# SewoongLab/PLeaS-Merging

Measured on AMD Instinct MI355X. Metric: wall-clock (s): ResNet-101 pair, 100-batch act-match + 400-step PLeaS, 1/8 GPU, lower is better.
Workload: dtype f32

## Files before the change

include/pleas_hip.h:

```cpp
#ifndef PLEAS_HIP_H
#define PLEAS_HIP_H

#include <stddef.h>
#include <stdint.h>

#ifdef __cplusplus
extern "C" {
#endif

#define PLEAS_OK 0
#define PLEAS_EINVAL (-22)
#define PLEAS_ENOMEM (-12)
#define PLEAS_EHIP (-5)

const char* pleas_version(void);
const char* pleas_last_error(void);

#define PLEAS_EPI_INNER 0
#define PLEAS_EPI_NEG_CDIST 1
size_t pleas_gram_ws_bytes(int B, int C, int64_t HW);
int pleas_gram_accum(const float* x, const float* y, int B, int C, int64_t HW, int epilogue, int accumulate,
                     float* acc, void* ws, size_t ws_bytes, void* stream);

typedef struct pleas_gram_node {
// ... 6 lines not shown
    int derived;
    int source;
    const float* scale_x;
    const float* shift_x;
    const float* scale_y;
    const float* shift_y;
} pleas_gram_node;
size_t pleas_gram_batch_ws_bytes(const pleas_gram_node* nodes, int n_nodes, const int* group_C, int n_groups);
int pleas_gram_batch(const pleas_gram_node* nodes, int n_nodes, float* const* group_acc, const int* group_C,
                     int n_groups, int epilogue, int accumulate, void* ws, size_t ws_bytes, int ws_fresh, void* stream);

#define PLEAS_LSAP_MAX_N 4096
int pleas_lsap_batched(const float* const* cost, const int* n, int nprob, int maximize, int64_t* const* col_ind,
                       void* stream);
int pleas_lsap_host(const void* cost, int is_double, int n, int maximize, int64_t* col_ind);

size_t pleas_bottleneck_ws_bytes(const int* n, int nprob);
int pleas_bottleneck_batched(const float* const* cost, const int* n, int nprob, int maximize, int64_t* const* col_ind,
                             float* t_out, void* ws, size_t ws_bytes, void* stream);
int pleas_bottleneck_host(const void* cost, int is_double, int n, int maximize, int64_t* col_ind, double* t_out);

int pleas_merge_blocks(const float* w1, const float* w2, float* out, int64_t outer, int rows_out, int cols_out,
                       int64_t inner, int rows_src, int cols_src, const int32_t* row1, const int32_t* row2,
                       const int32_t* col1, const int32_t* col2, int n_merged_rows, void* stream);

typedef struct pleas_merge_item {
    const float* w1;
    const float* w2;
    float* out;
    const int32_t* row1;
    const int32_t* row2;
    int64_t outer, inner;
    int rows_out, rows_src, n_merged;
    int sub_stride, sub_h, sub_w;
} pleas_merge_item;
size_t pleas_merge_batch_ws_bytes(const pleas_merge_item* items, int n_items);
int pleas_merge_batch(const pleas_merge_item* items, int n_items, void* ws, size_t ws_bytes, int ws_fresh, void* stream);

int pleas_bn_act(const float* x, const float* scale, const float* shift, const float* res, float* y, int64_t n,
                 int channels, int64_t inner, int relu, void* stream);
int pleas_bn_act_tracked(const float* x, const float* scale, const float* shift, const float* res, float* y_bn,
                         float* y_sum, float* y, int64_t n, int channels, int64_t inner, int relu, void* stream);

int pleas_bn_act_tracked_batches(const float* x, const float* scale, const float* shift, const float* res, float* y_bn,
                                 float* y_sum, float* y, int64_t n_per_batch, int batches, int channels, int64_t inner,
                                 int relu, void* stream);

int pleas_bn_act_maxpool(const float* x, const float* scale, const float* shift, float* y, int64_t n, int channels, int H,
                         int W, int KH, int KW, int stride, int pad, int relu, void* stream);

size_t pleas_bn_train_ws_bytes(int64_t n, int channels);
int pleas_bn_train_fold(const float* x, int64_t n, int channels, int64_t inner, const float* gamma, const float* beta,
                        double eps, double momentum, float* running_mean, float* running_var,
                        int64_t* num_batches_tracked, float* scale, float* shift, void* ws, size_t ws_bytes,
                        void* stream);
int pleas_bn_train_fold_batches(const float* x, int64_t n, int batches, int channels, int64_t inner, const float* gamma,
                                const float* beta, double eps, double momentum, float* running_mean, float* running_var,
                                int64_t* num_batches_tracked, float* scale, float* shift, void* ws, size_t ws_bytes,
                                void* stream);

int pleas_masked_adam(float* p, const float* g, const float* mask, float* m, float* v, int64_t n, float lr,
                      float b1, float b2, float eps, int step, void* stream);

size_t pleas_sqerr_ws_bytes(int64_t n);
int pleas_sqerr(const float* a, const float* b, int64_t n, float scale, int accumulate, float* out, float dscale,
                float* diff, void* ws, size_t ws_bytes, void* stream);

int pleas_channel_sum(const float* x, int N, int C, int64_t HW, float* out, void* stream);

typedef struct pleas_fwd_layer {
    const float* ip;
    const float* w;
    const float* bias;
    const float* o1;
    const float* o2;
    const int32_t* row1;
    const int32_t* row2;
    float* resid;
    int N, Cout, Cin, Hin, Win, KH, KW, stride, pad, Csrc, n_merged;
    float dscale, loss_scale;
    int flags;
} pleas_fwd_layer;
#define PLEAS_FWD_KPOS_MAJOR 1
size_t pleas_fwd_batch_ws_bytes(const pleas_fwd_layer* layers, int n_layers);
int pleas_fwd_plan_lanes(double* form_ms, int* form_lane, int* form_items);
int pleas_fwd_plan_units(const pleas_fwd_layer* layers, int n_layers, const double* form_ms, int* units, int max_units);
int pleas_fwd_batch(const pleas_fwd_layer* layers, int n_layers, float* loss, void* ws, size_t ws_bytes, int ws_fresh,
                    void* stream);
int pleas_conv2d_fwd(const float* x, const float* w, const float* bias, float* y, int N, int Cin, int Hin, int Win, int Cout,
                     int KH, int KW, int stride, int pad, int flags, void* stream);
int pleas_conv2d_bn_act_fwd(const float* x, const float* w, const float* bias, float* y, const float* scale,
                            const float* shift, const float* res, float* z, int relu, int N, int Cin, int Hin, int Win,
                            int Cout, int KH, int KW, int stride, int pad, int flags, void* stream);
typedef struct pleas_wgrad_layer {
    const float* resid;
    const float* ip;
    float* grad;
    int N, Cout, Cin, Hin, Win, KH, KW, stride, pad;
    int flags;
} pleas_wgrad_layer;
#define PLEAS_WGRAD_ACCUMULATE 1
#define PLEAS_WGRAD_KPOS_MAJOR 2
int pleas_target_residual(const float* out, const float* o1, const float* o2, const int32_t* row1, const int32_t* row2,
                          int n_merged, int N, int C, int Csrc, int64_t HW, float dscale, float* resid, float* partials,
                          int* n_partials, void* stream);
int pleas_target_residual_max_partials(void);
int pleas_loss_final(const float* partials, const int* n_partials, const float* scale, int stride, int n_layers,
                     float* loss, void* stream);
size_t pleas_wgrad_batch_ws_bytes(const pleas_wgrad_layer* layers, int n_layers);
int pleas_wgrad_batch(const pleas_wgrad_layer* layers, int n_layers, void* ws, size_t ws_bytes, int ws_fresh,
                      void* stream);
int pleas_wgrad_plan_info(const pleas_wgrad_layer* layers, int n_layers, int* info);

int pleas_allreduce_sum(float* buf, int64_t n, void* comm, void* stream);

typedef struct pleas_neq_layer {
    const float* ip;
    float* A;
    int N, Cin, Hin, Win, KH, KW, stride, pad;
} pleas_neq_layer;
size_t pleas_normal_eq_ws_bytes(const pleas_neq_layer* layers, int n_layers);
int pleas_normal_eq_accum(const pleas_neq_layer* layers, int n_layers, void* ws, size_t ws_bytes, int ws_fresh,
                          void* stream);
int pleas_normal_eq_finalize(const pleas_neq_layer* layers, int n_layers, void* stream);
int pleas_normal_eq_plan_info(const pleas_neq_layer* layers, int n_layers, double* info);

int pleas_cholesky_solve_batched(float* const* A, float* const* Bt, const int* K, const int* N, int nprob, float lambda,
                                 int* info, void* stream);

void pleas_prof_enable(int on);
void pleas_prof_select(unsigned kernel_mask);
void pleas_prof_reset(void);
int pleas_prof_collect(int kernel, int64_t* launches, double* total_ms, double* flops, double* bytes);

void pleas_gram_tune(int target_blocks, int min_chunks_per_split);
void pleas_gram_batch_tune(int item_chunks, int xcd_order);
#define PLEAS_ARITH_FP32 0
#define PLEAS_ARITH_SPLIT_BF16 1
void pleas_arith(int mode);
int pleas_arith_get(void);
void pleas_gram_split_bf16(int on);
void pleas_wgrad_tune(int item_chunks);

#ifdef __cplusplus
}
#endif
#endif
```

pleas_merging_amd/csrc/conv_fwd.hip:

```cpp
#include <algorithm>
#include <mutex>
#include <vector>

#include "common.hpp"
#include "fwd_schedule.hpp"

namespace pleas {

typedef float f32x4 __attribute__((ext_vector_type(4)));
typedef float f32x16 __attribute__((ext_vector_type(16)));

constexpr int fBK = 32;
constexpr int fLdsA = 36;
constexpr int fLdsB = 36;
constexpr int fTN = 128;
constexpr int fThreads = 256;

struct FwdLayerDev {
    const float* ip;
    const float* w;
    const float* bias;
    const float* o1;
    const float* o2;
    const int32_t* row1;
// ... 692 lines not shown
        store_a((c + 1) & 1, ra_next);
        if (newb) {
            if constexpr (NBUF == 2) {
                bsel ^= 1;
                store_b(bsel, rb_next);
            } else {
                __syncthreads();
                store_b(0, rb0);
            }
        }
        __syncthreads();
        r1 = r2;
        cb1 = cb2;
    };
    int r = 0;
    int c = 0;
    for (; c + 2 < nchunks; c += 2) {
        const int ra_ = r1;
        step(c, r, ra1, ra0, rb1, rb0);
        const int rb_ = r1;
        step(c + 1, ra_, ra0, ra1, rb0, rb1);
        r = rb_;
    }
    if (c + 1 < nchunks) {
        const int ra_ = r1;
        step(c, r, ra1, ra0, rb1, rb0);
        r = ra_;
    }
    fwd_load_maps<TM, PLAIN>(L, i0, m1, m2, bias_v);
    compute((nchunks - 1) & 1, bsel, r);
    __syncthreads();
    fwd_epilogue<TM, PLAIN>(L, it, acc, m1, m2, bias_v, smem, partials);
}

struct FwdForm {
    bool flat;
    int tm;
    int sub;
    bool split;
    int occupancy[2];
    double weight;
};
constexpr int fForms = 10;
constexpr FwdForm kFwdForms[fForms] = {
    {false, 128, 4, false, {2, 2}, 2.5}, {false, 64, 4, false, {2, 2}, 2.5},
    {false, 128, 1, false, {2, 2}, 2.5}, {false, 64, 1, false, {2, 2}, 2.5},
    {true, 128, 0, true, {2, 2}, 1.0},   {true, 128, 1, false, {2, 2}, 2.0}, {true, 128, 2, true, {2, 2}, 1.0},
    {true, 64, 0, true, {2, 3}, 1.0},    {true, 64, 1, false, {2, 2}, 2.0},  {true, 64, 2, true, {2, 3}, 1.0},
};
constexpr int fwd_form_of(int variant) {
    if (variant & 8) return ((variant & 1) ? 7 : 4) + ((variant >> 4) & 3);
    return variant & 3;
}
constexpr bool fwd_forms_match_variants() {
    for (int f = 0; f < fForms; ++f) {
        const FwdForm& F = kFwdForms[f];
        const int variant = (F.tm == 64 ? 1 : 0) | (F.flat ? 8 | (F.sub << 4) : (F.sub == 1 ? 2 : 0));
        if (fwd_form_of(variant) != f || (F.split && !(F.flat && F.sub != 1))) return false;
    }
    return true;
}
static_assert(fwd_forms_match_variants(), "kFwdForms is indexed by the form id");
template <int FORM, int SPLIT = 0>
__global__ __launch_bounds__(fThreads, kFwdForms[FORM].occupancy[SPLIT]) void fwd_batch_kernel(const FwdLayerDev* __restrict__ layers,
                                                             const FwdItemDev* __restrict__ items,
                                                             float* __restrict__ partials) {
    extern __shared__ __attribute__((aligned(16))) float smem[];
    const FwdItemDev it = items[blockIdx.x];
    if (it.layer < 0) return;
    const FwdLayerDev L = layers[it.layer];
    constexpr FwdForm F = kFwdForms[FORM];
    if constexpr (F.flat) fwd_flat_tile<F.tm, F.sub, SPLIT>(L, it, smem, partials);
    else fwd_tile<F.tm, F.sub>(L, it, smem, partials);
}
template <int FORM, int SPLIT = 0, int BN = 0>
__global__ __launch_bounds__(fThreads, kFwdForms[FORM].occupancy[SPLIT]) void conv2d_fwd_kernel(const FwdLayerDev L, const int tms) {
    extern __shared__ __attribute__((aligned(16))) float smem[];
    const FwdItemDev it{0, (int)(blockIdx.x % (unsigned)tms), (int)(blockIdx.x / (unsigned)tms), 0};
    constexpr FwdForm F = kFwdForms[FORM];
    constexpr int PLAIN = 1 + BN;
    if constexpr (F.flat) fwd_flat_tile<F.tm, F.sub, SPLIT, PLAIN>(L, it, smem, nullptr);
    else fwd_tile<F.tm, F.sub, PLAIN>(L, it, smem, nullptr);
}
struct FwdFormKernels {
    void (*batch[2])(const FwdLayerDev*, const FwdItemDev*, float*);
    void (*conv2d[2][2])(const FwdLayerDev, const int);
};
template <int FORM>
static constexpr FwdFormKernels fwd_form_kernels() {
    constexpr int S = kFwdForms[FORM].split ? 1 : 0;
    return {{fwd_batch_kernel<FORM, 0>, fwd_batch_kernel<FORM, S>},
            {{conv2d_fwd_kernel<FORM, 0, 0>, conv2d_fwd_kernel<FORM, S, 0>}, {conv2d_fwd_kernel<FORM, 0, 1>, conv2d_fwd_kernel<FORM, S, 1>}}};
}
static const FwdFormKernels kFwdKernels[fForms] = {fwd_form_kernels<0>(), fwd_form_kernels<1>(), fwd_form_kernels<2>(), fwd_form_kernels<3>(),
                                                   fwd_form_kernels<4>(), fwd_form_kernels<5>(), fwd_form_kernels<6>(), fwd_form_kernels<7>(),
                                                   fwd_form_kernels<8>(), fwd_form_kernels<9>()};
constexpr int fLanes = 3;
static SideStreams<fLanes> g_fwd_side;

struct FwdLossDev {
    int begin, count;
    float scale;
    int pad;
};
__global__ __launch_bounds__(64) void fwd_loss_kernel(const float* __restrict__ partials, const FwdLossDev* __restrict__ ld,
                                                      float* __restrict__ loss) {
    const FwdLossDev d = ld[blockIdx.x];
    double s = 0.0;
    for (int i = threadIdx.x; i < d.count; i += 64) s += (double)partials[d.begin + i];
#pragma unroll
    for (int off = 32; off >= 1; off >>= 1) s += __shfl_xor(s, off);
    if (threadIdx.x == 0) loss[blockIdx.x] = (float)(s * (double)d.scale);
}

constexpr int fPtrBatch = 56;
struct FwdPtrBatch {
    int base, count;
    const float* ip[fPtrBatch];
    const float* w[fPtrBatch];
    const float* bias[fPtrBatch];
    const float* o1[fPtrBatch];
    const float* o2[fPtrBatch];
    const int32_t* row1[fPtrBatch];
    const int32_t* row2[fPtrBatch];
    float* resid[fPtrBatch];
};
__global__ void fwd_set_ptrs_kernel(FwdLayerDev* __restrict__ layers, const FwdPtrBatch b) {
    const int t = blockIdx.x * blockDim.x + threadIdx.x;
    if (t < b.count) {
        FwdLayerDev& L = layers[b.base + t];
        L.ip = b.ip[t];
        L.w = b.w[t];
        L.bias = b.bias[t];
        L.o1 = b.o1[t];
        L.o2 = b.o2[t];
        L.row1 = b.row1[t];
        L.row2 = b.row2[t];
        L.resid = b.resid[t];
    }
}

struct FwdPlan {
    std::vector<int64_t> key;
    std::vector<FwdLayerDev> layers;
    std::vector<FwdItemDev> items;
    std::vector<FwdLossDev> loss;
    size_t off_layers = 0, off_items = 0, off_loss = 0, off_parts = 0, total = 0;
    int form_begin[fForms] = {0}, form_count[fForms] = {0};
    size_t form_lds[fForms] = {0};
    std::vector<float> item_work;
    std::vector<FwdUnit> units;
    double flops = 0, bytes = 0;
    int n_parts = 0;
    bool uploaded = false;
    bool split = false;
    int launches = 0, calib = 0;
    hipEvent_t t0[kFwdMaxUnits], t1[kFwdMaxUnits];
    int timed = 0;
    bool timing_events() {
        if (timed == 0) {
            timed = 1;
            for (int u = 0; u < kFwdMaxUnits && timed == 1; ++u)
                if (hipEventCreate(&t0[u]) != hipSuccess || hipEventCreate(&t1[u]) != hipSuccess) timed = -1;
        }
        return timed == 1;
    }
// ... 83 lines not shown
        P.form_lds[form] = std::max(P.form_lds[form], lds_bytes);
        P.flops += 2.0 * l.Cout * (double)Kd * (double)Ptot;
        P.bytes += ((double)l.Cin * l.N * l.Hin * l.Win + 3.0 * l.Cout * (double)Ptot) * sizeof(float);
    }
    for (int f = 0; f < fForms; ++f) {
        P.form_begin[f] = (int)P.items.size();
        std::vector<FwdItemDev> part = xcd_order_items(work[f], FwdItemDev{-1, 0, 0, 0}, false);
        P.items.insert(P.items.end(), part.begin(), part.end());
        P.form_count[f] = (int)part.size();
    }
    P.item_work.assign(P.items.size(), 0.f);
    for (size_t k = 0; k < P.items.size(); ++k)
        if (P.items[k].layer >= 0) {
            const FwdLayerDev& d = P.layers[P.items[k].layer];
            P.item_work[k] = (float)(ceil_div(d.Kd, fBK) * kFwdForms[fwd_form_of(d.variant)].tm);
        }
    P.units.clear();
    for (int f = 0; f < fForms; ++f)
        if (P.form_count[f] > 0)
            P.units.push_back(FwdUnit{f, P.form_begin[f], P.form_count[f], 0, form_work[f] * kFwdForms[f].weight});
    fwd_deal_lanes(P.units, fLanes + 1);
    P.launches = P.calib = 0;
    P.n_parts = parts;
    size_t off = 0;
    P.off_layers = off;
    off = align256(off + P.layers.size() * sizeof(FwdLayerDev));
    P.off_items = off;
    off = align256(off + P.items.size() * sizeof(FwdItemDev));
    P.off_loss = off;
    off = align256(off + P.loss.size() * sizeof(FwdLossDev));
    P.off_parts = off;
    P.total = off + (size_t)parts * sizeof(float);
    P.uploaded = false;
    return PLEAS_OK;
}

}

using namespace pleas;

extern "C" int pleas_fwd_plan_lanes(double* form_ms, int* form_lane, int* form_items) {
    if (!form_ms || !form_lane || !form_items) return bad_arg("fwd_plan_lanes: null pointer");
    std::lock_guard<std::mutex> lk(g_fplan_mu);
    if (!g_fplans.last) return bad_arg("fwd_plan_lanes: no grouped forward has run yet");
    const FwdPlan& P = *g_fplans.last;
    for (int f = 0; f < fForms; ++f) {
        form_ms[f] = 0;
        form_lane[f] = 0;
        form_items[f] = P.form_count[f];
    }
    for (const auto& u : P.units) {
        form_ms[u.form] += u.ms;
        form_lane[u.form] = form_lane[u.form] * 10 + u.lane + 1;
    }
    return P.calib;
}

extern "C" int pleas_fwd_plan_units(const pleas_fwd_layer* layers, int n_layers, const double* form_ms, int* units, int max_units) {
    if (!layers || n_layers <= 0 || !units || max_units <= 0) return bad_arg("fwd_plan_units: empty layer list / null output");
    FwdPlan tmp;
    const int rc = build_fwd_plan(tmp, layers, n_layers);
    if (rc != PLEAS_OK) return rc;
    if (form_ms) {
        for (auto& u : tmp.units) u.ms = form_ms[u.form];
        (void)fwd_schedule_measured(tmp.units, tmp.form_items(), fLanes + 1, kFwdMaxUnits);
    }
    const int n = (int)std::min<size_t>(tmp.units.size(), (size_t)max_units);
    for (int i = 0; i < n; ++i) {
        units[4 * i + 0] = tmp.units[i].form;
        units[4 * i + 1] = tmp.units[i].begin;
        units[4 * i + 2] = tmp.units[i].count;
        units[4 * i + 3] = tmp.units[i].lane;
    }
    return (int)tmp.units.size();
}

extern "C" size_t pleas_fwd_batch_ws_bytes(const pleas_fwd_layer* layers, int n_layers) {
    if (!layers || n_layers <= 0) return 0;
    FwdPlan tmp;
    if (build_fwd_plan(tmp, layers, n_layers) != PLEAS_OK) return 0;
    return tmp.total;
}

static int conv2d_launch(const float* x, const float* w, const float* bias, float* y, const float* scale, const float* shift,
                         const float* res, float* z, int relu, int N, int Cin, int Hin, int Win, int Cout, int KH, int KW,
                         int stride, int pad, int flags, void* stream_) {
    if (!x || !w || !y) return bad_arg("conv2d_fwd: null pointer");
    if (((uintptr_t)w & 15) != 0 || ((uintptr_t)x & 15) != 0) return bad_arg("conv2d_fwd: x and w must be 16-byte aligned");
    const bool bn = scale != nullptr;
    if (bn && (!shift || !z)) return bad_arg("conv2d_bn_act_fwd: scale needs shift and z");
    if (bn && ((((uintptr_t)y | (uintptr_t)z | (uintptr_t)res) & 15) != 0))
        return bad_arg("conv2d_bn_act_fwd: y, z and res must be 16-byte aligned");
    pleas_fwd_layer l{};
    l.ip = x; l.w = w; l.bias = bias; l.resid = y;
    l.N = N; l.Cout = Cout; l.Cin = Cin; l.Hin = Hin; l.Win = Win; l.KH = KH; l.KW = KW; l.stride = stride; l.pad = pad;
    l.Csrc = 1; l.n_merged = 0; l.dscale = 1.f; l.loss_scale = 0.f; l.flags = flags;
    FwdLayerDev d{};
    size_t lds = 0;
    int TM = 128;
    if (const int rc = fwd_describe(l, d, lds, TM); rc != PLEAS_OK) return rc;
    d.ip = x; d.w = w; d.bias = bias; d.o1 = x; d.o2 = x; d.row1 = nullptr; d.row2 = nullptr; d.resid = y;
    d.part_base = 0;
    d.bn_scale = scale; d.bn_shift = shift; d.bn_res = res; d.bn_z = z; d.bn_relu = relu ? 1 : 0;
    const int tms = (int)ceil_div(Cout, TM), tps = (int)ceil_div((int64_t)d.Ptot, fTN);
    const dim3 grid((unsigned)((int64_t)tms * tps));
    hipStream_t st = (hipStream_t)stream_;
    const double out_floats = (double)Cout * d.Ptot;
    ProfScope prof(kProfConv2d, 2.0 * Cout * (double)d.Kd * (double)d.Ptot,
                   ((double)Cin * N * Hin * Win + out_floats * (bn ? (res ? 3.0 : 2.0) : 1.0)) * sizeof(float), st);
    hipLaunchKernelGGL(kFwdKernels[fwd_form_of(d.variant)].conv2d[bn ? 1 : 0][arith_mode() == 1 ? 1 : 0], grid, dim3(fThreads), lds, st, d, tms);
    PLEAS_LAUNCH_CHECK("conv2d_fwd_kernel");
    return PLEAS_OK;
}

extern "C" int pleas_conv2d_fwd(const float* x, const float* w, const float* bias, float* y, int N, int Cin, int Hin, int Win,
                                int Cout, int KH, int KW, int stride, int pad, int flags, void* stream_) {
    return conv2d_launch(x, w, bias, y, nullptr, nullptr, nullptr, nullptr, 0, N, Cin, Hin, Win, Cout, KH, KW, stride, pad, flags,
                         stream_);
}

extern "C" int pleas_conv2d_bn_act_fwd(const float* x, const float* w, const float* bias, float* y, const float* scale,
                                       const float* shift, const float* res, float* z, int relu, int N, int Cin, int Hin,
                                       int Win, int Cout, int KH, int KW, int stride, int pad, int flags, void* stream_) {
    if (!scale || !shift || !z) return bad_arg("conv2d_bn_act_fwd: null pointer");
    return conv2d_launch(x, w, bias, y, scale, shift, res, z, relu, N, Cin, Hin, Win, Cout, KH, KW, stride, pad, flags, stream_);
}

static void fwd_adopt_measurements(FwdPlan& P) {
    if (P.calib != 1) return;
    const int active = (int)P.units.size();
    bool ready = true;
    for (int u = 0; ready && u < active; ++u) ready = hipEventQuery(P.t1[u]) == hipSuccess;
    if (ready) {
        for (int u = 0; u < active; ++u) {
            float ms = 0.f;
            P.units[u].ms = hipEventElapsedTime(&ms, P.t0[u], P.t1[u]) == hipSuccess ? ms : 0.0;
        }
        P.calib = 2;
        if (fwd_schedule_measured(P.units, P.form_items(), fLanes + 1, kFwdMaxUnits))
            g_fcalib.publish(P.key, P.units);
    }
    (void)hipGetLastError();
}

static int fwd_launch_units(FwdPlan& P, const FwdLayerDev* dl, const FwdItemDev* items, float* parts, hipStream_t stream) {
    ProfScope prof(kProfConvFwd, P.flops, P.bytes, stream);
    SideStreams<fLanes>::Set& side = g_fwd_side.current();
    const int active = (int)P.units.size();
    const bool fork = active > 1 && side.ok;
    const bool measure = fork && P.calib == 0 && P.launches == kFwdCalibAt && active <= kFwdMaxUnits && P.timing_events();
    if (fork) PLEAS_HIP_CHECK(hipEventRecord(side.forked, stream));
    bool lane_used[fLanes + 1] = {false};
    for (int o = 0; o < active; ++o) {
        const FwdUnit& un = P.units[o];
        const int lane = fork ? un.lane : 0;
        hipStream_t st = lane == 0 ? stream : side.streams[lane - 1];
        if (lane > 0 && !lane_used[lane]) PLEAS_HIP_CHECK(hipStreamWaitEvent(st, side.forked, 0));
        lane_used[lane] = true;
        if (measure) PLEAS_HIP_CHECK(hipEventRecord(P.t0[o], st));
        hipLaunchKernelGGL(kFwdKernels[un.form].batch[P.split ? 1 : 0], dim3((unsigned)un.count), dim3(fThreads), P.form_lds[un.form], st,
                           dl, items + un.begin, parts);
        if (measure) PLEAS_HIP_CHECK(hipEventRecord(P.t1[o], st));
    }
    if (measure) P.calib = 1;
    for (int lane = 1; lane <= fLanes; ++lane)
        if (lane_used[lane]) {
            PLEAS_HIP_CHECK(hipEventRecord(side.joined[lane - 1], side.streams[lane - 1]));
            PLEAS_HIP_CHECK(hipStreamWaitEvent(stream, side.joined[lane - 1], 0));
        }
    return PLEAS_OK;
}

extern "C" int pleas_fwd_batch(const pleas_fwd_layer* layers, int n_layers, float* loss, void* ws, size_t ws_bytes,
                               int ws_fresh, void* stream_) {
    if (!layers || n_layers <= 0 || !loss) return bad_arg("conv_fwd: empty layer list");
    for (int i = 0; i < n_layers; ++i) {
        const pleas_fwd_layer& l = layers[i];
        if (!l.ip || !l.w || !l.o1 || !l.o2 || !l.row1 || !l.row2 || !l.resid) return bad_arg("conv_fwd: null pointer");
        if (((uintptr_t)l.w & 15) != 0) return bad_arg("conv_fwd: weights must be 16-byte aligned");
        if (((uintptr_t)l.ip & 15) != 0) return bad_arg("conv_fwd: the merged input must be 16-byte aligned");
    }
    hipStream_t stream = (hipStream_t)stream_;
    std::lock_guard<std::mutex> lk(g_fplan_mu);
    std::vector<int64_t> key;
    key.push_back(n_layers * 2 + arith_mode());
    key.push_back((int64_t)(uintptr_t)ws);
    for (int i = 0; i < n_layers; ++i) {
        const pleas_fwd_layer& l = layers[i];
        for (int v : {l.N, l.Cout, l.Cin, l.Hin, l.Win, l.KH, l.KW, l.stride, l.pad, l.Csrc, l.n_merged, l.flags})
            key.push_back(v);
        int32_t bits[2];
        std::memcpy(&bits[0], &l.dscale, 4);
// ... 45 lines not shown
```

pleas_merging_amd/hip_ops.py:

```python
from __future__ import annotations

import ctypes
import math
import threading
from typing import List, Optional, Sequence, Tuple

import numpy as np
import torch

from . import _lib
from ._lib import EPI_INNER, EPI_NEG_CDIST, PleasHipError, check


class _Pinned(threading.local):

    depth = 0
    handle = 0


_PINNED = _Pinned()


def _stream() -> int:
    if _PINNED.depth > 0:
# ... 581 lines not shown
    rc = _lib.lib().pleas_loss_final(partials.data_ptr(), n_partials.data_ptr(), scale.data_ptr(), stride, L,
                                     loss.data_ptr(), _stream())
    check(rc, "pleas_loss_final")


class MergeBatch(_GroupedLaunch):

    STRUCT, WS_BYTES, LAUNCH = _lib.MergeItem, "pleas_merge_batch_ws_bytes", "pleas_merge_batch"

    def add(self, w1: torch.Tensor, w2: torch.Tensor, row_axis: int, row1: torch.Tensor, row2: torch.Tensor,
            n_merged_rows: int, out: Optional[torch.Tensor] = None, subsample: int = 1) -> torch.Tensor:
        if w1.shape != w2.shape or not w1.is_cuda or w1.dtype != torch.float32 or w2.dtype != torch.float32:
            raise PleasHipError("MergeBatch.add: fp32 CUDA sources of equal shape expected")
        w1, w2 = w1.contiguous(), w2.contiguous()
        shape = list(w1.shape)
        row_axis = row_axis % w1.dim()
        rows_out = int(row1.numel())
        want = shape[:row_axis] + [rows_out] + shape[row_axis + 1:]
        sub = (0, 0, 0)
        if subsample > 1:
            if w1.dim() != 4 or row_axis != 1:
                raise PleasHipError("MergeBatch.add: subsample needs [N, C, H, W] sources merged along axis 1")
            sub = (int(subsample), shape[2], shape[3])
            want = want[:2] + [-(-shape[2] // subsample), -(-shape[3] // subsample)]
        if out is None:
            out = torch.empty(want, dtype=torch.float32, device=w1.device)
        elif list(out.shape) != want or out.dtype != torch.float32 or not out.is_contiguous() or out.device != w1.device:
            raise PleasHipError("MergeBatch.add: out must be a contiguous fp32 tensor of shape %s" % (want,))
        self._queue((w1, w2, out, row1, row2), (math.prod(shape[:row_axis]), math.prod(want[row_axis + 1:]), rows_out,
                                                shape[row_axis], int(n_merged_rows)) + sub)
        return out

    def _fill(self, a, tensors, geo) -> None:
        a.w1, a.w2, a.out, a.row1, a.row2 = (t.data_ptr() for t in tensors)
        a.outer, a.inner, a.rows_out, a.rows_src, a.n_merged, a.sub_stride, a.sub_h, a.sub_w = geo


def fwd_plan_lanes() -> dict:
    ms, lane, items = (ctypes.c_double * 10)(), (ctypes.c_int * 10)(), (ctypes.c_int * 10)()
    state = _lib.lib().pleas_fwd_plan_lanes(ms, lane, items)
    return {"state": state, "forms": {f: {"ms": round(ms[f], 4), "lane": lane[f], "items": items[f]} for f in range(10) if items[f]}}


class FwdBatch(_GroupedLaunch):

    STRUCT, WS_BYTES, LAUNCH = _lib.FwdLayer, "pleas_fwd_batch_ws_bytes", "pleas_fwd_batch"
    KPOS_MAJOR = 1

    def add(self, ip, w, bias, o1, o2, row1, row2, n_merged: int, resid, dscale: float, loss_scale: float,
            kernel=(1, 1), stride: int = 1, pad: int = 0, flags: int = 0) -> None:
        for t in (ip, w, o1, o2, resid):
            if not t.is_contiguous():
                raise PleasHipError("FwdBatch.add: contiguous tensors expected")
        N, Cin = ip.shape[0], ip.shape[1]
        Hin, Win = (ip.shape[2], ip.shape[3]) if ip.dim() == 4 else (1, 1)
        self._queue((ip, w, bias, o1, o2, row1, row2, resid),
                    (N, w.shape[0], Cin, Hin, Win, kernel[0], kernel[1], stride, pad, o1.shape[1], int(n_merged),
                     float(dscale), float(loss_scale), int(flags)))

    def _fill(self, a, tensors, geo) -> None:
        a.ip, a.w, a.bias, a.o1, a.o2, a.row1, a.row2, a.resid = (t.data_ptr() if t is not None else None for t in tensors)
        (a.N, a.Cout, a.Cin, a.Hin, a.Win, a.KH, a.KW, a.stride, a.pad, a.Csrc, a.n_merged, a.dscale, a.loss_scale,
         a.flags) = geo

    def _launch_args(self, loss: torch.Tensor) -> tuple:
        if loss.numel() != len(self._arr) or not loss.is_contiguous():
            raise PleasHipError("FwdBatch: loss must hold one float per layer")
        return (loss.data_ptr(),)

    def flush(self, loss: torch.Tensor) -> None:
        self._flush(loss)


def _conv_geometry(name: str, x: torch.Tensor, w: torch.Tensor, stride: int, pad: int, kpos_major: bool):
    if x.dim() != 4 or w.dim() != 4 or not x.is_contiguous() or not w.is_contiguous():
        raise PleasHipError("%s: contiguous 4-D tensors expected" % name)
    N, Cin, H, W = x.shape
    KH, KW = (w.shape[1], w.shape[2]) if kpos_major else (w.shape[2], w.shape[3])
    if (w.shape[3] if kpos_major else w.shape[1]) != Cin:
        raise PleasHipError("%s: %d input channels vs a weight of %s" % (name, Cin, tuple(w.shape)))
    return N, Cin, H, W, w.shape[0], KH, KW, (H + 2 * pad - KH) // stride + 1, (W + 2 * pad - KW) // stride + 1


def conv2d(x: torch.Tensor, w: torch.Tensor, bias: Optional[torch.Tensor], stride: int, pad: int, kpos_major: bool = False,
           out: Optional[torch.Tensor] = None) -> torch.Tensor:
    _need_gpu(x, w)
    N, Cin, H, W, Cout, KH, KW, Ho, Wo = _conv_geometry("conv2d", x, w, stride, pad, kpos_major)
    if out is None:
        out = torch.empty((N, Cout, Ho, Wo), dtype=torch.float32, device=x.device)
    check(_lib.lib().pleas_conv2d_fwd(x.data_ptr(), w.data_ptr(), bias.data_ptr() if bias is not None else None, out.data_ptr(),
                                      N, Cin, H, W, Cout, KH, KW, stride, pad, FwdBatch.KPOS_MAJOR if kpos_major else 0,
                                      _stream()), "pleas_conv2d_fwd")
    return out


def conv2d_bn_act(x: torch.Tensor, w: torch.Tensor, bias: Optional[torch.Tensor], stride: int, pad: int, kpos_major: bool,
                  scale: torch.Tensor, shift: torch.Tensor, res: Optional[torch.Tensor], relu: bool):
    _need_gpu(x, w, scale, shift)
    N, Cin, H, W, Cout, KH, KW, Ho, Wo = _conv_geometry("conv2d_bn_act", x, w, stride, pad, kpos_major)
    if scale.numel() != Cout or shift.numel() != Cout or scale.dtype != torch.float32 or shift.dtype != torch.float32:
        raise PleasHipError("conv2d_bn_act: scale / shift must be fp32 vectors of %d channels" % Cout)
    if res is not None and (tuple(res.shape) != (N, Cout, Ho, Wo) or res.dtype != torch.float32 or not res.is_contiguous()
                            or res.device != x.device):
        raise PleasHipError("conv2d_bn_act: the identity must be a contiguous fp32 tensor shaped like the output")
    y = torch.empty((N, Cout, Ho, Wo), dtype=torch.float32, device=x.device)
    z = torch.empty_like(y)
    check(_lib.lib().pleas_conv2d_bn_act_fwd(x.data_ptr(), w.data_ptr(), bias.data_ptr() if bias is not None else None,
                                             y.data_ptr(), scale.data_ptr(), shift.data_ptr(),
                                             res.data_ptr() if res is not None else None, z.data_ptr(), 1 if relu else 0,
                                             N, Cin, H, W, Cout, KH, KW, stride, pad,
                                             FwdBatch.KPOS_MAJOR if kpos_major else 0, _stream()), "pleas_conv2d_bn_act_fwd")
    return y, z


class WgradBatch(_GroupedLaunch):

    STRUCT, WS_BYTES, LAUNCH = _lib.WgradLayer, "pleas_wgrad_batch_ws_bytes", "pleas_wgrad_batch"
    ACCUMULATE, KPOS_MAJOR = 1, 2

    def add(self, resid: torch.Tensor, ip: torch.Tensor, grad: torch.Tensor, kernel=(1, 1), stride: int = 1,
            pad: int = 0, flags: int = 0) -> None:
        if not (resid.is_contiguous() and ip.is_contiguous() and grad.is_contiguous()):
            raise PleasHipError("WgradBatch.add: contiguous tensors expected")
        N, Cout, Cin = resid.shape[0], resid.shape[1], ip.shape[1]
        Hin, Win = (ip.shape[2], ip.shape[3]) if ip.dim() == 4 else (1, 1)
        self._queue((resid, ip, grad), (N, Cout, Cin, Hin, Win, kernel[0], kernel[1], stride, pad, flags))

    def _fill(self, a, tensors, geo) -> None:
        a.resid, a.ip, a.grad = (t.data_ptr() for t in tensors)
        a.N, a.Cout, a.Cin, a.Hin, a.Win, a.KH, a.KW, a.stride, a.pad, a.flags = geo

    @staticmethod
    def plan_info(geometries) -> List[dict]:
        geometries = list(geometries)
        n = len(geometries)
        if n == 0:
            return []
        arr = (_lib.WgradLayer * n)()
        for a, geo in zip(arr, geometries):
            a.N, a.Cout, a.Cin, a.Hin, a.Win, a.KH, a.KW, a.stride, a.pad, a.flags = (int(v) for v in geo)
        info = (ctypes.c_int * (6 * n))()
        check(_lib.lib().pleas_wgrad_plan_info(arr, n, info), "pleas_wgrad_plan_info")
        return [{"variant": info[6 * i], "S": info[6 * i + 1], "tiles_cout": info[6 * i + 2], "tiles_cin": info[6 * i + 3],
                 "items": info[6 * i + 4], "rows": bool(info[6 * i + 5])} for i in range(n)]

class NormalEqBatch(_GroupedLaunch):

    STRUCT, WS_BYTES, LAUNCH = _lib.NeqLayer, "pleas_normal_eq_ws_bytes", "pleas_normal_eq_accum"

    def __init__(self, device: torch.device):
        super().__init__(device)
        self._seen: dict = {}

    def add(self, ip: torch.Tensor, A: torch.Tensor, kernel=(1, 1), stride: int = 1, pad: int = 0) -> None:
        if not (ip.is_contiguous() and A.is_contiguous()):
            raise PleasHipError("NormalEqBatch.add: contiguous tensors expected")
        N, Cin = ip.shape[0], ip.shape[1]
        Hin, Win = (ip.shape[2], ip.shape[3]) if ip.dim() == 4 else (1, 1)
        K = kernel[0] * kernel[1] * Cin
        if tuple(A.shape) != (K, K):
            raise PleasHipError("NormalEqBatch.add: A must be (%d, %d)" % (K, K))
        geo = (N, Cin, Hin, Win, kernel[0], kernel[1], stride, pad)
        self._queue((ip, A), geo)
        self._seen[A.data_ptr()] = (A, geo)

    def _fill(self, a, tensors, geo) -> None:
        ip, A = tensors
        a.ip, a.A = (ip.data_ptr() if ip is not None else 0), A.data_ptr()
        a.N, a.Cin, a.Hin, a.Win, a.KH, a.KW, a.stride, a.pad = geo

    def _layer_array(self, pairs):
        arr = (_lib.NeqLayer * len(pairs))()
        for a, (A, geo) in zip(arr, pairs):
            self._fill(a, (None, A), geo)
        return arr

    def seen(self) -> dict:
        return dict(self._seen)

    def finalize(self, pairs=None) -> None:
        pairs = list(self._seen.values()) if pairs is None else list(pairs)
        if pairs:
            check(_lib.lib().pleas_normal_eq_finalize(self._layer_array(pairs), len(pairs), _stream()),
                  "pleas_normal_eq_finalize")

    def plan_info(self) -> dict:
        pairs = list(self._seen.values())
        info = (ctypes.c_double * 4)()
        if pairs:
            check(_lib.lib().pleas_normal_eq_plan_info(self._layer_array(pairs), len(pairs), info), "pleas_normal_eq_plan_info")
        return {"flops": info[0], "flops_executed": info[1], "items": int(info[2]), "blocks_to_finalize": int(info[3])}


def cholesky_solve_batched(As: Sequence[torch.Tensor], Bts: Sequence[torch.Tensor], ridge: float = 0.0) -> torch.Tensor:
# ... 39 lines not shown
```

Before: 5.857.

## Add persistent weight-resident streaming kernel for 1x1 conv forward

Adds a persistent conv2d forward kernel for 1x1 flat convolutions with Cin up to 256. It keeps a whole Cout tile of weights in LDS and streams pixel tiles through a double-buffered register and LDS pipeline, with the bias/BN/residual/ReLU epilogue fused in. The grid is sized to the number of resident workgroups from an occupancy query, so weights are loaded once per workgroup rather than once per tile. The aim is to cut repeated weight traffic and launch tail effects. The cost is heavy LDS use, lower occupancy, and a path that is on by default for matching shapes.

```diff
diff --git a/include/pleas_hip.h b/include/pleas_hip.h
--- a/include/pleas_hip.h
+++ b/include/pleas_hip.h
@@ -112,6 +112,10 @@
     int flags;
 } pleas_fwd_layer;
 #define PLEAS_FWD_KPOS_MAJOR 1
+#define PLEAS_FWD_NO_STREAM 2
+#define PLEAS_FWD_STREAM_ALT_TM 4
+#define PLEAS_FWD_STREAM_GRID_SHIFT 8
+#define PLEAS_FWD_STREAM_GRID(n) (((n) & 0xffff) << PLEAS_FWD_STREAM_GRID_SHIFT)
 size_t pleas_fwd_batch_ws_bytes(const pleas_fwd_layer* layers, int n_layers);
 int pleas_fwd_plan_lanes(double* form_ms, int* form_lane, int* form_items);
 int pleas_fwd_plan_units(const pleas_fwd_layer* layers, int n_layers, const double* form_ms, int* units, int max_units);
diff --git a/pleas_merging_amd/csrc/conv_fwd.hip b/pleas_merging_amd/csrc/conv_fwd.hip
--- a/pleas_merging_amd/csrc/conv_fwd.hip
+++ b/pleas_merging_amd/csrc/conv_fwd.hip
@@ -798,6 +798,204 @@
     if constexpr (F.flat) fwd_flat_tile<F.tm, F.sub, SPLIT, PLAIN>(L, it, smem, nullptr);
     else fwd_tile<F.tm, F.sub, PLAIN>(L, it, smem, nullptr);
 }
+constexpr int fStreamMaxCin = 256;
+constexpr int fStreamLdsBudget = 160 * 1024;
+constexpr size_t fwd_stream_lds(int TM, int Cin) {
+    return (size_t)(TM * (Cin + 4) + 2 * fBK * fFlatRow1 + TM * 132) * sizeof(float);
+}
+template <int TM, int BN>
+__global__ __launch_bounds__(fThreads, TM == 64 ? 2 : 1) void conv2d_stream_kernel(const FwdLayerDev L, const int tms, const int tps, const int runs) {
+    extern __shared__ __attribute__((aligned(16))) float smem[];
+    constexpr int MTM = TM / 64, ROWS = TM / 8, Lr = fFlatRow1, EL = 132;
+    const int tid = threadIdx.x, lane = tid & 63, wave = tid >> 6;
+    const int wm = wave >> 1, wn = wave & 1;
+    int tm = (int)(blockIdx.x % (unsigned)tms), run = (int)(blockIdx.x / (unsigned)tms);
+    if (runs % 8 == 0) {
+        const int s = (int)(blockIdx.x >> 3);
+        tm = s % tms;
+        run = (s / tms) * 8 + (int)(blockIdx.x & 7);
+    }
+    const int t0 = (int)((int64_t)run * tps / runs), t1 = (int)((int64_t)(run + 1) * tps / runs);
+    if (t0 == t1) return;
+    const int i0 = tm * TM;
+    const int CB = L.Cin / fBK, WS = L.Cin + 4;
+    const uint32_t HW = L.HWo, hw4 = 4u * HW;
+    float* Ws = smem;
+    float* Bs = Ws + TM * WS;
+    float* Ct = Bs + 2 * fBK * Lr;
+    {
+        const int q4 = L.Cin / 4;
+        for (int idx = tid; idx < TM * q4; idx += fThreads) {
+            const int row = idx / q4, c4 = idx - row * q4;
+            const int gi = i0 + row;
+            f32x4 v = *(const __attribute__((address_space(1))) f32x4*)(PLEAS_GLOBAL(L.w) + (uint32_t)min(gi, L.Cout - 1) * L.Kd + 4 * c4);
+            if (gi >= L.Cout) v = f32x4{0.f, 0.f, 0.f, 0.f};
+            *reinterpret_cast<f32x4*>(Ws + row * WS + 4 * c4) = v;
+        }
+    }
+    const int r8 = tid >> 5, pg = (tid & 31) * 4;
+    float bias_v[ROWS], sc[ROWS], sh[ROWS];
+#pragma unroll
+    for (int j = 0; j < ROWS; ++j) {
+        const int co = min(i0 + r8 + 8 * j, L.Cout - 1);
+        bias_v[j] = L.bias ? PLEAS_GLOBAL(L.bias)[co] : 0.f;
+        sc[j] = BN ? PLEAS_GLOBAL(L.bn_scale)[co] : 0.f;
+        sh[j] = BN ? PLEAS_GLOBAL(L.bn_shift)[co] : 0.f;
+    }
+    auto tile_group = [&](int t, uint32_t& n, uint32_t& p) {
+        const uint32_t P4 = (uint32_t)t * fTN + (uint32_t)pg;
+        const bool ok = P4 < L.Ptot;
+        n = ok ? P4 / HW : 0u;
+        p = ok ? P4 - n * HW : 0u;
+        return ok;
+    };
+    int lt = t0, lcb = 0;
+    uint32_t lvoff = 0;
+    bool lvok = false;
+    auto cursor_tile = [&]() {
+        uint32_t n, p;
+        lvok = tile_group(lt, n, p);
+        lvoff = lvok ? n * (uint32_t)L.Cin * HW + p + (uint32_t)r8 * HW : 0u;
+    };
+    auto load_b = [&](float (&rb)[16], bool& vok) {
+        const cgfloat* base = PLEAS_GLOBAL(L.ip) + (size_t)lcb * fBK * HW;
+#pragma unroll
+        for (int i = 0; i < 4; ++i) {
+            const f32x4 v = *(const __attribute__((address_space(1))) f32x4*)(base + lvoff + (uint32_t)(8 * i) * HW);
+#pragma unroll
+            for (int e = 0; e < 4; ++e) rb[4 * i + e] = v[e];
+        }
+        vok = lvok;
+        if (++lcb == CB) {
+            lcb = 0;
+            ++lt;
+            cursor_tile();
+        }
+    };
+    auto store_b = [&](int buf, const float (&rb)[16], bool vok) {
+        float* b = Bs + buf * fBK * Lr;
+#pragma unroll
+        for (int i = 0; i < 4; ++i) {
+            const f32x4 v = {vok ? rb[4 * i] : 0.f, vok ? rb[4 * i + 1] : 0.f, vok ? rb[4 * i + 2] : 0.f, vok ? rb[4 * i + 3] : 0.f};
+            *reinterpret_cast<f32x4*>(b + (r8 + 8 * i) * Lr + pg) = v;
+        }
+    };
+    f32x16 acc[MTM][2];
+    auto zero_acc = [&]() {
+#pragma unroll
+        for (int a = 0; a < MTM; ++a)
+#pragma unroll
+            for (int b = 0; b < 2; ++b)
+#pragma unroll
+                for (int r = 0; r < 16; ++r) acc[a][b][r] = 0.f;
+    };
+    auto compute = [&](int buf, int cb) {
+        const float* a = Ws + (wm * (TM / 2) + (lane & 31)) * WS + cb * fBK + 4 * (lane >> 5);
+        const float* b0 = Bs + buf * fBK * Lr + 4 * (lane >> 5) * Lr + wn * 64 + (lane & 31);
+        const float* b1 = b0 + 32;
+#pragma unroll
+        for (int kk = 0; kk < fBK / 8; ++kk) {
+            f32x4 fa[MTM];
+#pragma unroll
+            for (int s = 0; s < MTM; ++s) fa[s] = *reinterpret_cast<const f32x4*>(a + s * 32 * WS + kk * 8);
+#pragma unroll
+            for (int e = 0; e < 4; ++e) {
+                const float f0 = b0[(kk * 8 + e) * Lr], f1 = b1[(kk * 8 + e) * Lr];
+#pragma unroll
+                for (int sm = 0; sm < MTM; ++sm) {
+                    acc[sm][0] = __builtin_amdgcn_mfma_f32_32x32x2f32(fa[sm][e], f0, acc[sm][0], 0, 0, 0);
+                    acc[sm][1] = __builtin_amdgcn_mfma_f32_32x32x2f32(fa[sm][e], f1, acc[sm][1], 0, 0, 0);
+                }
+            }
+        }
+    };
+    const bool has_res = BN && L.bn_res != nullptr;
+    const char* idb = reinterpret_cast<const char*>(has_res ? L.bn_res : L.ip);
+    char* yb = reinterpret_cast<char*>(L.resid);
+    char* zb = reinterpret_cast<char*>(L.bn_z);
+    bool gin = false;
+    uint32_t rbase = 0;
+    f32x4 ta[BN ? ROWS : 1];
+    auto open_tile = [&](int t) {
+        uint32_t n, p;
+        gin = tile_group(t, n, p);
+        rbase = 4u * ((n * (uint32_t)L.Cout + (uint32_t)(i0 + r8)) * HW + p);
+        if constexpr (BN) {
+#pragma unroll
+            for (int j = 0; j < ROWS; ++j) {
+                const bool live = has_res && gin && i0 + r8 + 8 * j < L.Cout;
+                const uint32_t oz = live ? rbase + (uint32_t)(8 * j) * hw4 : 0u;
+                const f32x4 idn = *(const __attribute__((address_space(1))) f32x4*)(idb + oz);
+                ta[j] = has_res ? idn : f32x4{0.f, 0.f, 0.f, 0.f};
+            }
+        }
+    };
+    auto close_tile = [&]() {
+#pragma unroll
+        for (int sm = 0; sm < MTM; ++sm)
+#pragma unroll
+            for (int sn = 0; sn < 2; ++sn)
+#pragma unroll
+                for (int r = 0; r < 16; ++r) {
+                    const int lco = wm * (TM / 2) + sm * 32 + (r & 3) + 8 * (r >> 2) + 4 * (lane >> 5);
+                    Ct[lco * EL + wn * 64 + sn * 32 + (lane & 31)] = acc[sm][sn][r];
+                }
+        zero_acc();
+        __syncthreads();
+#pragma unroll
+        for (int j = 0; j < ROWS; ++j) {
+            const int lco = r8 + 8 * j;
+            const bool live = gin && i0 + lco < L.Cout;
+            const f32x4 o = *reinterpret_cast<const f32x4*>(Ct + lco * EL + pg);
+            const uint32_t at = rbase + (uint32_t)(8 * j) * hw4;
+            f32x4 y, z;
+#pragma unroll
+            for (int e = 0; e < 4; ++e) {
+                y[e] = o[e] + bias_v[j];
+                if constexpr (BN) {
+                    const float s = fmaf(y[e], sc[j], sh[j]) + ta[j][e];
+                    z[e] = L.bn_relu ? fmaxf(s, 0.f) : s;
+                }
+            }
+            if (live) {
+                *(__attribute__((address_space(1))) f32x4*)(yb + at) = y;
+                if constexpr (BN) *(__attribute__((address_space(1))) f32x4*)(zb + at) = z;
+            }
+        }
+    };
+
+    const int total = (t1 - t0) * CB;
+    float rb0[16], rb1[16];
+    bool vk0 = false, vk1 = false;
+    cursor_tile();
+    load_b(rb0, vk0);
+    if (total > 1) load_b(rb1, vk1);
+    zero_acc();
+    store_b(0, rb0, vk0);
+    __syncthreads();
+    int g = 0, ct = t0, ccb = 0;
+    auto step = [&](float (&rb_next)[16], bool& vk_next, float (&rb_far)[16], bool& vk_far) {
+        if (g + 2 < total) load_b(rb_far, vk_far);
+        if (ccb == 0) open_tile(ct);
+        compute(g & 1, ccb);
+        if (g + 1 < total) store_b((g + 1) & 1, rb_next, vk_next);
+        __syncthreads();
+        if (++ccb == CB) {
+            close_tile();
+            ccb = 0;
+            ++ct;
+        }
+    };
+    for (;;) {
+        step(rb1, vk1, rb0, vk0);
+        if (++g == total) break;
+        step(rb0, vk0, rb1, vk1);
+        if (++g == total) break;
+    }
+}
+static void (*const kStreamKernels[2][2])(const FwdLayerDev, const int, const int, const int) = {
+    {conv2d_stream_kernel<64, 0>, conv2d_stream_kernel<64, 1>}, {conv2d_stream_kernel<128, 0>, conv2d_stream_kernel<128, 1>}};
+
 struct FwdFormKernels {
     void (*batch[2])(const FwdLayerDev*, const FwdItemDev*, float*);
     void (*conv2d[2][2])(const FwdLayerDev, const int);
@@ -1047,6 +1245,26 @@
     return tmp.total;
 }
 
+static int stream_resident_groups(int tm128, int bn, size_t lds) {
+    static std::mutex mu;
+    static std::vector<std::pair<std::vector<int64_t>, int>> known;
+    int dev = 0;
+    if (hipGetDevice(&dev) != hipSuccess) return 0;
+    const std::vector<int64_t> key{dev, tm128, bn, (int64_t)lds};
+    std::lock_guard<std::mutex> lk(mu);
+    for (const auto& k : known)
+        if (k.first == key) return k.second;
+    const void* fn = reinterpret_cast<const void*>(kStreamKernels[tm128][bn]);
+    int cus = 0, per_cu = 0;
+    (void)hipFuncSetAttribute(fn, hipFuncAttributeMaxDynamicSharedMemorySize, fStreamLdsBudget);
+    if (lds > (size_t)fStreamLdsBudget || hipDeviceGetAttribute(&cus, hipDeviceAttributeMultiprocessorCount, dev) != hipSuccess ||
+        hipOccupancyMaxActiveBlocksPerMultiprocessor(&per_cu, fn, fThreads, lds) != hipSuccess)
+        cus = per_cu = 0;
+    (void)hipGetLastError();
+    known.emplace_back(key, cus * per_cu);
+    return cus * per_cu;
+}
+
 static int conv2d_launch(const float* x, const float* w, const float* bias, float* y, const float* scale, const float* shift,
                          const float* res, float* z, int relu, int N, int Cin, int Hin, int Win, int Cout, int KH, int KW,
                          int stride, int pad, int flags, void* stream_) {
@@ -1073,6 +1291,23 @@
     const double out_floats = (double)Cout * d.Ptot;
     ProfScope prof(kProfConv2d, 2.0 * Cout * (double)d.Kd * (double)d.Ptot,
                    ((double)Cin * N * Hin * Win + out_floats * (bn ? (res ? 3.0 : 2.0) : 1.0)) * sizeof(float), st);
+    if (!(flags & PLEAS_FWD_NO_STREAM) && arith_mode() == 0 && (d.variant & 8) && ((d.variant >> 4) & 3) == 0 && Cin <= fStreamMaxCin) {
+        const bool can128 = Cout > 64 && fwd_stream_lds(128, Cin) <= (size_t)fStreamLdsBudget;
+        const int tm128 = (can128 && (flags & PLEAS_FWD_STREAM_ALT_TM)) ? 1 : 0;
+        const int sTM = tm128 ? 128 : 64;
+        const size_t slds = fwd_stream_lds(sTM, Cin);
+        int groups = stream_resident_groups(tm128, bn ? 1 : 0, slds);
+        const int cap = (flags >> PLEAS_FWD_STREAM_GRID_SHIFT) & 0xffff;
+        if (cap > 0) groups = std::min(groups, cap);
+        if (groups > 0) {
+            const int stms = (int)ceil_div(Cout, sTM);
+            int runs = std::max(1, groups / stms);
+            if (runs >= 32) runs &= ~7;
+            hipLaunchKernelGGL(kStreamKernels[tm128][bn ? 1 : 0], dim3((unsigned)(stms * runs)), dim3(fThreads), slds, st, d, stms, tps, runs);
+            PLEAS_LAUNCH_CHECK("conv2d_stream_kernel");
+            return PLEAS_OK;
+        }
+    }
     hipLaunchKernelGGL(kFwdKernels[fwd_form_of(d.variant)].conv2d[bn ? 1 : 0][arith_mode() == 1 ? 1 : 0], grid, dim3(fThreads), lds, st, d, tms);
     PLEAS_LAUNCH_CHECK("conv2d_fwd_kernel");
     return PLEAS_OK;
diff --git a/pleas_merging_amd/hip_ops.py b/pleas_merging_amd/hip_ops.py
--- a/pleas_merging_amd/hip_ops.py
+++ b/pleas_merging_amd/hip_ops.py
@@ -687,20 +687,27 @@
     return N, Cin, H, W, w.shape[0], KH, KW, (H + 2 * pad - KH) // stride + 1, (W + 2 * pad - KW) // stride + 1
 
 
+CONV_NO_STREAM, CONV_STREAM_ALT_TM = 2, 4
+
+
+def conv_stream_grid(workgroups: int) -> int:
+    return (int(workgroups) & 0xffff) << 8
+
+
 def conv2d(x: torch.Tensor, w: torch.Tensor, bias: Optional[torch.Tensor], stride: int, pad: int, kpos_major: bool = False,
-           out: Optional[torch.Tensor] = None) -> torch.Tensor:
+           out: Optional[torch.Tensor] = None, flags: int = 0) -> torch.Tensor:
     _need_gpu(x, w)
     N, Cin, H, W, Cout, KH, KW, Ho, Wo = _conv_geometry("conv2d", x, w, stride, pad, kpos_major)
     if out is None:
         out = torch.empty((N, Cout, Ho, Wo), dtype=torch.float32, device=x.device)
     check(_lib.lib().pleas_conv2d_fwd(x.data_ptr(), w.data_ptr(), bias.data_ptr() if bias is not None else None, out.data_ptr(),
-                                      N, Cin, H, W, Cout, KH, KW, stride, pad, FwdBatch.KPOS_MAJOR if kpos_major else 0,
-                                      _stream()), "pleas_conv2d_fwd")
+                                      N, Cin, H, W, Cout, KH, KW, stride, pad,
+                                      (FwdBatch.KPOS_MAJOR if kpos_major else 0) | int(flags), _stream()), "pleas_conv2d_fwd")
     return out
 
 
 def conv2d_bn_act(x: torch.Tensor, w: torch.Tensor, bias: Optional[torch.Tensor], stride: int, pad: int, kpos_major: bool,
-                  scale: torch.Tensor, shift: torch.Tensor, res: Optional[torch.Tensor], relu: bool):
+                  scale: torch.Tensor, shift: torch.Tensor, res: Optional[torch.Tensor], relu: bool, flags: int = 0):
     _need_gpu(x, w, scale, shift)
     N, Cin, H, W, Cout, KH, KW, Ho, Wo = _conv_geometry("conv2d_bn_act", x, w, stride, pad, kpos_major)
     if scale.numel() != Cout or shift.numel() != Cout or scale.dtype != torch.float32 or shift.dtype != torch.float32:
@@ -714,7 +721,8 @@
                                              y.data_ptr(), scale.data_ptr(), shift.data_ptr(),
                                              res.data_ptr() if res is not None else None, z.data_ptr(), 1 if relu else 0,
                                              N, Cin, H, W, Cout, KH, KW, stride, pad,
-                                             FwdBatch.KPOS_MAJOR if kpos_major else 0, _stream()), "pleas_conv2d_bn_act_fwd")
+                                             (FwdBatch.KPOS_MAJOR if kpos_major else 0) | int(flags), _stream()),
+          "pleas_conv2d_bn_act_fwd")
     return y, z
 
 
```

After: 5.881. About the same (+0.4%).
